# DINT-NSDI24/DINT

Hardware: AMD Instinct MI355X
Metric: Mtxn/s + p50/p99 batch latency, TATP (higher is better)
Workload: dtype u64

## Files before the change

### dint_amd/csrc/k_kv_dev.h

```cpp
#pragma once
#include <algorithm>
#include <cstddef>
#include <cstdlib>
#include <cstring>
#include <utility>
#include <vector>

#include "../../include/dint_abi.h"
#include "dint_kv.h"
#define KVB_SORT_INLINE
#include "dint_bins.h"
#include "log_ring.h"

template <int WL> struct Fmt;
template <> struct Fmt<DINT_WL_STORE> {
  static constexpr uint32_t MSG = 53, TYPE = 0, KEY = 1, VAL = 9, VER = 49, VS = 40;
  static constexpr bool HAS_TABLE = false;
  static constexpr uint32_t TABLE = 0;
};
template <> struct Fmt<DINT_WL_TATP> {
  static constexpr uint32_t MSG = 55, TYPE = 1, KEY = 3, VAL = 11, VER = 51, VS = 40;
  static constexpr bool HAS_TABLE = true;
  static constexpr uint32_t TABLE = 2;
};
// ... 2012 lines not shown
            uint32_t pos;
            if (fancy) {
              const int lw = top(mW & below), lwb = top((mW | mB) & below);
              const uint32_t w = wc + (uint32_t)__popcll(mW & below);
              const uint32_t jj = (lw < 0 ? jc : 0u) + (uint32_t)__popcll(mB & below & above(lw));
              const uint64_t mine = q == 0 ? mA[0] : q == 1 ? mA[1] : q == 2 ? mA[2] : mA[3];
              const bool follows = (mine & below & above(lwb)) != 0 || (lwb < 0 && ((af >> q) & 1u));
              pos = w * stride + (cl == 0 ? 0u : cl == 1 ? 3u * jj + (follows ? 1u : 0u) : cl == 2 ? 3u * jj + 2u : stride - 1u);
            } else {
              pos = 2u * (vc + (uint32_t)__popcll(mV & below)) + (cl ? 1u : 0u);
            }
            if (valid) Rpos[p] = (uint16_t)pos;
            const int tw = top(mW), twb = top(mW | mB);
            wc += (uint32_t)__popcll(mW);
            jc = (tw < 0 ? jc : 0u) + (uint32_t)__popcll(mB & above(tw));
            if (twb >= 0) af = 0;
#pragma unroll
            for (uint32_t i = 0; i < 4; i++) af |= (mA[i] & above(twb)) ? 1u << i : 0u;
            vc += (uint32_t)__popcll(mV);
          }
        }
      }
    }
    __syncthreads();
    for (uint32_t j = 0; j < ntile; j++) {
      const uint32_t p = j * KVB_T + t;
      const uint32_t pos = p < m ? Rpos[p] : 0xFFFFu;
      if (pos != 0xFFFFu) atomicOr(&Rbits[pos >> 5], 1u << (pos & 31));
    }
    {
      uint32_t mx = mylen;
      for (int d = 32; d > 0; d >>= 1) mx = max(mx, (uint32_t)__shfl_xor(mx, d, 64));
      if (lane == 0) Sred[wave] = mx;
      __syncthreads();
      tot = 0;
      for (uint32_t w = 0; w < KVB_W; w++) tot = max(tot, Sred[w]);
    }
    for (uint32_t rw = 0; rw * 32 < tot; rw++) {
      for (uint32_t bits = Rbits[rw]; bits; bits &= bits - 1) {
        const uint32_t r = rw * 32 + (uint32_t)__ffs((int)bits) - 1;
        nrounds++;
        for (uint32_t j = 0; j < ntile; j++) {
          const uint32_t p = j * KVB_T + t;
          if (p < m && Rpos[p] == r) {
            const uint64_t cur = Sk[p];
            const uint32_t gk = kv_cut_gk((uint32_t)(cur >> sh_g), bin, cut), table = kv_table_of(kv, gk);
            kv_do_request<WL>(rep + dint_view_off(V, k_idx(cur), F::MSG), k_type(cur), table, k_q(cur),
                              (uint64_t)(gk - kv->gk_base[table]), kv, stats);
          }
        }
        __builtin_amdgcn_fence(__ATOMIC_SEQ_CST, "workgroup");
        __syncthreads();
      }
    }
    }
    if (wtr && t == 0) { wtr[14] += nrounds; wtr[15] += 1; }
    KVB_STAMP(13);
    __builtin_amdgcn_fence(__ATOMIC_SEQ_CST, "workgroup");
    __syncthreads();
  }
#undef KVB_STAMP
}

#define KVR_LCAP 1024u
#define KVR_F 64u
#define KVR_NPMAX 64u
struct kvr_lds {
  uint4 rec[KVR_LCAP];
  uint32_t hist[KVR_F];
  uint32_t cur[KVR_F];
  uint32_t off[KVR_F + 1];
  uint32_t bigoff[KVR_F];
  uint2 chs[KVR_F];
  uint32_t nch;
  uint32_t cflag[KVR_F];
  uint64_t ckey[KVR_F], hrec[KVR_F];
};
__device__ static inline uint32_t kv_piece_of(uint32_t idx, uint32_t np, uint32_t inv_n) {
  const uint32_t p = (uint32_t)(((uint64_t)idx * np * inv_n) >> 32);
  return p < np ? p : np - 1;
}
#define KVQ_W 3u
enum : uint32_t { KVQ_SUB = 0, KVQ_PIECE = 1, KVQ_REM = 2, KVQ_SOLO = 3 };

__device__ static inline void kv_list_items(const kv_pass_args &A, uint32_t b, const kvr_lds &L, const uint2 *Sbig) {
  const uint32_t t = threadIdx.x & 63u;
  const uint2 bs = Sbig[t];
  uint32_t target = A.split_target;
  if (A.V.seg_cap) {
    uint32_t live = t < A.V.n_seg ? min(A.V.seg_cap, *(const uint32_t *)(A.V.cnt + (size_t)t * A.V.cnt_stride)) : 0u, tot;
    (void)wave_excl_scan_u32(live, &tot);
    if (tot < A.n) target = max(8u, (uint32_t)(((uint64_t)target * max(tot, 1u)) / A.n));
  }
  const uint32_t np0 = (bs.y + target - 1) / target;
  const bool hot = bs.y >= A.split_min && np0 <= A.np_max;
  const uint32_t np = hot ? np0 : 0u;
  const uint32_t nent = bs.y ? (np > 1 ? np + 1 : 1u) : 0u;
  uint32_t tot, at = wave_excl_scan_u32(nent, &tot);
  uint32_t base = 0;
  if (t == 0 && tot) base = atomicAdd(&A.big[3], tot);
  base = (uint32_t)__builtin_amdgcn_readfirstlane((int)base);
  at += base;
  const uint32_t bin = b + A.cut.P * t;
  if (nent && !hot) {
    kv_st_agent(A.bigq + KVQ_W * (size_t)at, make_uint4(bin, bs.x, bs.y, KVQ_SUB));
  } else if (nent) {
    uint64_t hk = L.ckey[t], hr = L.hrec[t];
    if (A.sb_pieces) {
      using F = Fmt<DINT_WL_SMALLBANK>;
      const uint32_t sh_g = 16 + A.cut.ibits;
      uint64_t smp[8];
#pragma unroll
      for (uint32_t j = 0; j < 8; j++) smp[j] = kv_ld_agent(&A.ovf[bs.x + (uint32_t)(((uint64_t)(2 * j + 1) * bs.y) >> 4)]);
      uint32_t best = 0, bj = 0;
#pragma unroll
      for (uint32_t j = 0; j < 8; j++) {
        uint32_t c = 0;
#pragma unroll
        for (uint32_t i = 0; i < 8; i++) c += (smp[i] >> sh_g) == (smp[j] >> sh_g) && pay_q(kv_rec_pay(smp[i])) == pay_q(kv_rec_pay(smp[j]));
        if (c > best) { best = c; bj = j; }
      }
      hr = smp[0];
#pragma unroll
      for (uint32_t j = 1; j < 8; j++) if (j == bj) hr = smp[j];
      const uint32_t hidx = (uint32_t)(hr >> 16) & (uint32_t)((1ull << A.cut.ibits) - 1ull);
      hk = ld_u64(A.rep + dint_view_off(A.V, hidx, F::MSG) + F::KEY);
    }
    for (uint32_t p = 0; p < nent; p++) {
      const uint32_t kind = np == 1 ? KVQ_SOLO : (p < np ? KVQ_PIECE : KVQ_REM);
      uint4 *q = A.bigq + KVQ_W * (size_t)(at + p);
      kv_st_agent(q, make_uint4(bin, bs.x, bs.y, kind | (p << 2) | (np << 10)));
      kv_st_agent(q + 1, make_uint4((uint32_t)hk, (uint32_t)(hk >> 32), at, 0u));
      kv_st_agent(q + 2, make_uint4((uint32_t)hr, (uint32_t)(hr >> 32), 0u, 0u));
    }
  }
  asm volatile("s_waitcnt vmcnt(0)" ::: "memory");
  for (uint32_t p = 0; p < nent; p++)
    if (at + p < DINT_KV_BIGQ_MAX) __hip_atomic_store(&A.bigrdy[at + p], A.seq, __ATOMIC_RELAXED, __HIP_MEMORY_SCOPE_AGENT);
  asm volatile("s_waitcnt vmcnt(0)" ::: "memory");
  if (t == 0) atomicAdd(&A.big[6], 1u);
}

template <int WL, uint32_t NT>
__device__ static inline void kv_coarse_bin(const kv_pass_args &A, const kv_dev *kv, uint32_t coarse, uint8_t *lds_raw,
                                            uint2 *Sbig ,
                                            uint32_t cnt, const uint4 &r0, const uint4 &r1, uint64_t *tr) {
  kvr_lds &L = *(kvr_lds *)lds_raw;
  const uint32_t t = threadIdx.x, lane = t & 63, wave = t >> 6;
  const kv_cut &cut = A.cut;
  const uint32_t C = cut.P, cap = A.cap, sh = 16 + cut.ibits;
  const uint32_t idx_mask = (uint32_t)((1ull << cut.ibits) - 1ull);
  const uint4 *__restrict__ recs = A.kbins + (size_t)coarse * cap;
  if (cnt == 0) {
    if (t == 0) atomicAdd(&A.big[6], 1u);
    return;
  }
  const uint32_t n_in = min(cnt, cap);
  const uint32_t novl = cnt > cap ? A.big[1] : 0u;
  if (t == 0) A.bin_cnt[coarse] = 0;
  auto for_each_record = [&](auto &&f) {
    if (t < n_in) f(r0);
    if (t + NT < n_in) f(r1);
    for (uint32_t k0 = 2 * NT; k0 < n_in; k0 += 8 * NT) {
      uint4 q4[8];
#pragma unroll
      for (uint32_t j = 0; j < 8; j++) {
// ... 100 lines not shown
    const uint4 r = has ? L.rec[ab.x + lane] : make_uint4(0, 0, 0, 0);
    const uint64_t key0 = u4_key(r), m = u4_meta(r);
    const uint32_t pay0 = kv_rec_pay(m);
    uint64_t w = ~0ull;
    if (has) w = ((m >> sh) << (15 + cut.ibits)) | ((uint64_t)pay_kh(pay0) << (6 + cut.ibits)) | ((uint64_t)((uint32_t)(m >> 16) & idx_mask) << 6) | lane;
    w = wave_sort_u64(w);
    uint64_t *ctr = (tr && ch == 0) ? tr + 2 : nullptr;
    if (ctr && lane == 0) tr[5] = __builtin_amdgcn_s_memrealtime();
    const bool valid = lane < c;
    const int src = (int)((uint32_t)w & 63u);
    const uint64_t key = shfl_u64(key0, src);
    const uint32_t pay = (uint32_t)__shfl((int)pay0, src, 64);
    const uint32_t gk = kv_cut_gk((uint32_t)(w >> (15 + cut.ibits)), coarse, cut), kh = (uint32_t)(w >> (6 + cut.ibits)) & 511u;
    const uint32_t idx = (uint32_t)(w >> 6) & idx_mask;
    kv_chunk<WL>(A.rep, valid, valid ? idx : 0, gk, kh, pay_type(pay), valid ? kv_table_of(kv, gk) : 0, pay_q(pay), key, kv, A.stats,
                 A.force_flags & 1, true, A.V, ctr);
  }
}

template <int WL>
__device__ __forceinline__ static void kv_resolve_role(const kv_pass_args &A, uint32_t b, kv_dev &Skv, uint8_t *Lraw, uint2 *Sbig) {
  constexpr uint32_t NT = KVB_T;
  const uint32_t t = threadIdx.x;
  uint64_t *tr = A.trace ? A.trace + 32 * (size_t)b : nullptr;
  if (tr && t == 0) tr[0] = __builtin_amdgcn_s_memrealtime();
  static_assert(sizeof(kv_dev) / 4 <= NT, "one word of the table descriptors per thread");
  const uint4 *__restrict__ recs = A.kbins + (size_t)b * A.cap;
  const uint4 r0 = t < A.cap ? recs[t] : make_uint4(0, 0, 0, 0);
  const uint4 r1 = t + NT < A.cap ? recs[t + NT] : make_uint4(0, 0, 0, 0);
  const uint32_t kvw = t < sizeof(kv_dev) / 4 ? kv_dev_word(A.kv, A.big, t) : 0u;
  const uint32_t cnt = A.bin_cnt[b];
  if (t < sizeof(kv_dev) / 4) ((uint32_t *)&Skv)[t] = kvw;
  if (t < KVR_F) {
    Sbig[t] = make_uint2(0u, 0u);
    kvr_lds &L = *(kvr_lds *)Lraw;
    L.hist[t] = 0; L.cur[t] = 0; L.cflag[t] = 0;
  }
  if (b == 0) {
    if (t < 16 || (t >= KV_CTL_INS && t < KV_CTL_END)) A.big_z[t] = 0;
    for (uint32_t k = t; k < 1024; k += NT) A.blk_pub_z[k] = 0;
  }
  __syncthreads();
  kv_dev_pend_set(Skv, A.pno);
  if (tr && t == 0) tr[1] = __builtin_amdgcn_s_memrealtime();
  kv_coarse_bin<WL, NT>(A, &Skv, b, Lraw, Sbig, cnt, r0, r1, tr);
  if (tr && t == 0) { tr[11] = tr[12] = __builtin_amdgcn_s_memrealtime(); tr[13] = b; }
}
template <int WL>
__global__ void __launch_bounds__(KVB_T, 4) k_kv_resolve(kv_multi_args M, uint32_t n_eng) {
  __shared__ kv_dev Skv;
  __shared__ __attribute__((aligned(16))) uint8_t Lraw[sizeof(kvr_lds)];
  __shared__ uint2 Sbig[KVR_F];
  uint32_t e = 0, b = blockIdx.x;
  while (e + 1 < n_eng && b >= M.e[e].cut.P) { b -= M.e[e].cut.P; e++; }
  kv_resolve_role<WL>(M.e[e], b, Skv, Lraw, Sbig);
}

__device__ static inline unsigned long long kvh_word(uint32_t seq, bool ok, uint32_t nwr, int lw_idx, int ll_acq) {
  return ((unsigned long long)(seq & 0x3FFFFFFFu) << 34) | ((unsigned long long)(ok ? 1u : 0u) << 33) | ((unsigned long long)nwr << 23) |
         (lw_idx >= 0 ? (1ull << 22) | ((unsigned long long)(uint32_t)lw_idx << 2) : 0ull) | (ll_acq >= 0 ? 2ull | (unsigned long long)(ll_acq & 1) : 0ull);
}
struct kvh_lds {
  uint32_t key[KVB_T];
  uint32_t idx[KVB_T];
  uint8_t typ[KVB_T];
  uint64_t rem[KVB_T];
  uint64_t all[KVB_T];
  uint16_t cs[KVB_T + 2];
  uint64_t Bw[KVB_W], Bl[KVB_W], Ba[KVB_W];
  unsigned long long pub[KVR_NPMAX + 1];
  uint32_t bad, timeout, nhot, nrem, nall, nsame, nbr, nch, too_big;
  uint32_t found, link, slot, ver0, la0, table;
  uint32_t rowv[10];
  uint32_t best;
  unsigned long long hkey;
  uint32_t ev_ver[KVB_T];
  int16_t ev_src[KVB_T];
  uint8_t ev_ex[KVB_T];
  uint32_t fin_ex, fin_ver, fin_multi, fin_miss, dupf;
  int fin_src;
  uint8_t qq[KVB_T];
  uint64_t Lq[4][KVB_W], Aq[4][KVB_W];
  uint32_t lockw, bestg, gbad;
};
template <int WL>
__device__ __forceinline__ static bool kv_rem_chunks(uint8_t *rep, const kv_cut cut2, const kv_dev *kv, uint32_t bin, uint64_t *R, uint32_t m,
                                                     kvh_lds &H, dint_dev_stats *__restrict__ stats, int force_rounds, const dint_view V,
                                                     bool sorted = false ) {
  using F = Fmt<WL>;
  const uint32_t t = threadIdx.x, lane = t & 63, wave = t >> 6;
  const uint32_t sh_g = 16 + cut2.ibits, sh_k = 7 + cut2.ibits, idx_mask = (uint32_t)((1ull << cut2.ibits) - 1ull);
  __syncthreads();
  if (!sorted) {
    const uint64_t mine = t < m ? kv_sort_key(R[t], cut2) : ~0ull;
    __syncthreads();
    R[t] = mine;
    __syncthreads();
    uint32_t N = 64;
    while (N < m) N <<= 1;
    kvb_sort_blocked<1>(R, N);
  }
  const uint64_t w = R[t];
  const bool head = t < m && (t == 0 || (R[t - 1] >> sh_g) != (w >> sh_g));
  const uint64_t hm = __ballot(head);
  if (lane == 0) H.Bw[wave] = hm;
  __syncthreads();
  if (t == 0) {
    uint32_t nch = 0, start = 0, prev = 0, big = 0;
    for (uint32_t wv = 0; wv < KVB_W; wv++)
      for (uint64_t mm = H.Bw[wv]; mm; mm &= mm - 1) {
        const uint32_t hp = wv * 64 + (uint32_t)__ffsll((unsigned long long)mm) - 1;
        if (hp == 0) continue;
        if (hp - start > 64) { H.cs[nch++] = (uint16_t)start; start = prev; big |= hp - start > 64; }
        prev = hp;
      }
    if (m - start > 64) { H.cs[nch++] = (uint16_t)start; start = prev; big |= m - start > 64; }
    H.cs[nch++] = (uint16_t)start;
    H.cs[nch] = (uint16_t)m;
    H.nch = nch; H.too_big = big;
  }
  __syncthreads();
  if (H.too_big) return false;
  const uint32_t nch = H.nch;
  for (uint32_t ch = wave; ch < nch; ch += KVB_W) {
    const uint32_t a = H.cs[ch], c = H.cs[ch + 1] - a;
    const bool valid = lane < c;
    const uint64_t wv = valid ? R[a + lane] : ~0ull;
    const uint32_t idx = valid ? (uint32_t)(wv >> 7) & idx_mask : 0, gk = kv_cut_gk((uint32_t)(wv >> sh_g), bin, cut2);
    const uint32_t pay = (uint32_t)wv & 0x7Fu;
    const uint64_t key = valid ? ld_u64(rep + dint_view_off(V, idx, F::MSG) + F::KEY) : 0;
    kv_chunk<WL>(rep, valid, idx, gk, (uint32_t)(wv >> sh_k) & 511u, pay_type(pay), valid ? kv_table_of(kv, gk) : 0, pay_q(pay), key, kv, stats,
                 force_rounds, ch + KVB_W >= nch, V);
  }
  __builtin_amdgcn_fence(__ATOMIC_SEQ_CST, "workgroup");
  __syncthreads();
  return true;
}
#define KVG_MAXW 24u
template <int WL>
__device__ __forceinline__ static bool kv_group_phases(uint8_t *rep, const kv_cut cut2, const kv_dev *kv, uint32_t bin, const uint64_t *R, uint32_t Gs,
                                                       uint32_t Ge, kvh_lds &H, dint_dev_stats *__restrict__ stats, const dint_view V) {
  using F = Fmt<WL>;
  const uint32_t t = threadIdx.x, lane = t & 63, wave = t >> 6, n = Ge - Gs;
  const uint32_t sh_g = 16 + cut2.ibits, idx_mask = (uint32_t)((1ull << cut2.ibits) - 1ull);
  auto is_set = [](uint32_t type) -> bool { return WL == DINT_WL_STORE ? type == 1 : (type == 12 || type == 13); };
  auto is_ins = [](uint32_t type) -> bool { return WL == DINT_WL_STORE ? type == 2 : (type == 18 || type == 19); };
  auto is_del = [](uint32_t type) -> bool { return WL == DINT_WL_TATP && (type == 22 || type == 23); };
  const uint32_t gk = kv_cut_gk((uint32_t)(R[Gs] >> sh_g), bin, cut2), table = kv_table_of(kv, gk);
  const kv_tab tb = kv->tab[table];
  const uint64_t bucket = (uint64_t)(gk - kv->gk_base[table]);
  uint8_t *ie = kv_entry_ptr(tb, bucket, KV_INLINE);
  __syncthreads();
  {
    const uint64_t w = t < n ? R[Gs + t] : 0;
    const uint32_t idx = (uint32_t)(w >> 7) & idx_mask, pay = (uint32_t)w & 0x7Fu;
    H.key[t] = t < n ? (idx << 9) | t : 0xFFFFFFFFu;
    H.typ[t] = (uint8_t)(pay_type(pay) & 0xFFu);
    H.qq[t] = (uint8_t)pay_q(pay);
    H.rem[t] = t < n ? ld_u64(rep + dint_view_off(V, idx, F::MSG) + F::KEY) : 0;
    if (t == 0) { H.gbad = 0; H.lockw = KV_LD(uint32_t, ie + KV_LOCKB_OFF); }
  }
  __syncthreads();
  kvb_sort_blocked_u32<1>(H.key, KVB_T);
  const uint32_t sk = H.key[t];
  const bool v = sk != 0xFFFFFFFFu;
  const uint32_t slot = sk & 511u, my_idx = sk >> 9, my_type = v ? H.typ[slot] : 0xFFu, my_q = v ? H.qq[slot] : 0u;
// ... 70 lines not shown
      }
    }
  }
  __builtin_amdgcn_fence(__ATOMIC_SEQ_CST, "workgroup");
  __syncthreads();
  return true;
}
template <int WL>
__device__ __forceinline__ static int kv_solo_item(uint8_t *rep, const kv_cut cut2, const kv_dev *kv, const uint4 d,
                                                   const uint64_t *__restrict__ ovf, uint64_t *__restrict__ ovf2,
                                                   dint_dev_stats *__restrict__ stats, int force_rounds, const dint_view V, uint8_t *lds_raw,
                                                   uint32_t *src, uint32_t *off, uint32_t *cnt, uint64_t *ttr,
                                                   bool preloaded = false ) {
  using F = Fmt<WL>;
  kvh_lds &H = *(kvh_lds *)lds_raw;
  const uint32_t t = threadIdx.x, lane = t & 63, wave = t >> 6;
  const uint32_t h = d.z;
  const uint32_t sh_g = 16 + cut2.ibits, sh_k = 7 + cut2.ibits, idx_mask = (uint32_t)((1ull << cut2.ibits) - 1ull);
  *src = 0; *off = d.y; *cnt = h;
  if (h > KVB_T) return 1;
  auto is_set = [](uint32_t type) -> bool { return WL == DINT_WL_STORE ? type == 1 : (type == 12 || type == 13); };
  auto is_ins = [](uint32_t type) -> bool { return WL == DINT_WL_STORE ? type == 2 : (type == 18 || type == 19); };
  auto is_del = [](uint32_t type) -> bool { return WL == DINT_WL_TATP && (type == 22 || type == 23); };
  __syncthreads();
  if (!preloaded) H.all[t] = t < h ? kv_sort_key(kv_ld_agent(&ovf[d.y + t]), cut2) : ~0ull;
  if (t == 0) { H.bad = 0; H.best = 0; H.bestg = 0; H.dupf = 0; }
  __syncthreads();
  {
    uint32_t N = 64;
    while (N < h) N <<= 1;
    kvb_sort_blocked<1>(H.all, N);
  }
  const uint64_t w = H.all[t];
  const bool valid = t < h;
  const uint64_t prevw = t ? H.all[t - 1] : 0;
  const bool head_k = valid && (t == 0 || (prevw >> sh_k) != (w >> sh_k));
  const bool head_g = valid && (t == 0 || (prevw >> sh_g) != (w >> sh_g));
  const uint64_t mk = __ballot(head_k), mg = __ballot(head_g);
  if (lane == 0) { H.Bw[wave] = mk; H.Bl[wave] = mg; }
  __syncthreads();
  auto next_head = [&](const uint64_t *M) -> uint32_t {
    uint32_t nxt = h;
    for (uint32_t wv = wave; wv < KVB_W && nxt == h; wv++) {
      uint64_t mm = M[wv];
      if (wv == wave) mm &= ~((2ull << lane) - 1ull);
      if (mm) nxt = wv * 64 + (uint32_t)__ffsll((unsigned long long)mm) - 1;
    }
    return nxt;
  };
  if (head_k) atomicMax(&H.best, ((next_head(H.Bw) - t) << 16) | t);
  if (head_g) atomicMax(&H.bestg, ((next_head(H.Bl) - t) << 16) | t);
  __syncthreads();
  const uint32_t L = H.best >> 16, P = H.best & 0xFFFFu;
  uint32_t Gs = H.bestg & 0xFFFFu, Ge = Gs + (H.bestg >> 16);
  if (L > 64) {
    Gs = 0;
    for (uint32_t wv = 0; wv < KVB_W; wv++) {
      uint64_t mm = H.Bl[wv];
      if (wv * 64 > P) break;
      if (wv == (P >> 6)) mm &= (2ull << (P & 63)) - 1ull;
      if (mm) Gs = wv * 64 + 63 - (uint32_t)__clzll((long long)mm);
    }
    Ge = h;
    for (uint32_t wv = P >> 6; wv < KVB_W && Ge == h; wv++) {
      uint64_t mm = H.Bl[wv];
      if (wv == (P >> 6)) mm &= ~((2ull << (P & 63)) - 1ull);
      if (mm) Ge = wv * 64 + (uint32_t)__ffsll((unsigned long long)mm) - 1;
    }
  }
  auto rest = [&](uint32_t lo, uint32_t len) -> int {
    const uint32_t c_rem = h - len;
    if (c_rem == 0) return 0;
    __syncthreads();
    if (valid && (t < lo || t >= lo + len)) H.rem[t < lo ? t : t - len] = w;
    if (t >= c_rem) H.rem[t] = ~0ull;
    __builtin_amdgcn_fence(__ATOMIC_SEQ_CST, "workgroup");
    if (kv_rem_chunks<WL>(rep, cut2, kv, d.x, H.rem, c_rem, H, stats, force_rounds, V, true)) return 0;
    if (ovf2 && t < c_rem) {
      const uint64_t sw = H.rem[t];
      ovf2[d.y + t] = ((sw >> sh_g) << sh_g) | ((uint64_t)((uint32_t)(sw >> 7) & idx_mask) << 16) | ((uint32_t)sw & 0x7Fu) | (((uint32_t)(sw >> sh_k) & 511u) << 7);
    }
    __builtin_amdgcn_fence(__ATOMIC_SEQ_CST, "workgroup");
    *src = 1; *off = d.y; *cnt = c_rem;
    return 1;
  };
  auto phases = [&]() -> int {
    if (!kv_group_phases<WL>(rep, cut2, kv, d.x, H.all, Gs, Ge, H, stats, V)) return 1;
    return rest(Gs, Ge - Gs);
  };
  if (L <= 64) {
    if (ttr && t == 0) ttr[30] = (uint64_t)(d.w & 0xFFFFu) | (1ull << 17) | ((uint64_t)L << 20) | ((uint64_t)h << 32);
    if (Ge - Gs <= 64) return kv_rem_chunks<WL>(rep, cut2, kv, d.x, H.all, h, H, stats, force_rounds, V, true) ? 0 : 1;
    return phases();
  }
  const uint64_t hw = H.all[P];
  const uint32_t hq = pay_q((uint32_t)hw & 0x7Fu);
  const bool v = valid && t >= P && t < P + L;
  const uint32_t my_idx = (uint32_t)(w >> 7) & idx_mask, my_type = valid ? pay_type((uint32_t)w & 0x7Fu) : 0xFFu;
  if (valid && !v && (w >> sh_g) == (hw >> sh_g) && (kv_struct_op<WL>(my_type) || (kv_lock_op<WL>(my_type) && pay_q((uint32_t)w & 0x7Fu) == hq))) atomicOr(&H.bad, kv_struct_op<WL>(my_type) ? 1u : 2u);
  const uint64_t my_key = v ? ld_u64(rep + dint_view_off(V, my_idx, F::MSG) + F::KEY) : 0;
  if (t == P) H.hkey = my_key;
  const bool setop = v && is_set(my_type), insop = v && is_ins(my_type), delop = v && is_del(my_type);
  const bool lk = v && kv_lock_op<WL>(my_type), aq = v && WL == DINT_WL_TATP && my_type == 1;
  if (v && !(kv_simple_op<WL>(my_type) || kv_struct_op<WL>(my_type))) atomicOr(&H.bad, 4u);
  const uint64_t bev = __ballot(setop || insop || delop), bl = __ballot(lk), ba = __ballot(aq), bst = __ballot(insop || delop);
  if (lane == 0) { H.Bw[wave] = bev; H.Bl[wave] = bl; H.Ba[wave] = ba; }
  if (bst && lane == 0) H.dupf = 1;
  H.idx[t] = my_idx;
  H.typ[t] = (uint8_t)(my_type & 0xFFu);
  __syncthreads();
  const uint64_t hkey = H.hkey;
  if (v && my_key != hkey) atomicOr(&H.bad, 8u);
  const bool structural = H.dupf != 0;
  __syncthreads();
  kv_hdr Hd;
  kv_tab tb;
  uint64_t bucket = 0;
  uint32_t table = 0;
  {
    const uint32_t gk = kv_cut_gk((uint32_t)(hw >> sh_g), d.x, cut2);
    table = kv_table_of(kv, gk);
    tb = kv->tab[table];
    bucket = (uint64_t)(gk - kv->gk_base[table]);
  }
  if (t == P) {
    kv_hdr_load(Hd, kv_entry_ptr(tb, bucket, KV_INLINE));
    const kv_where wh = kv_locate(tb, bucket, Hd, hkey);
    H.found = wh.found; H.link = wh.link; H.slot = wh.slot; H.ver0 = wh.ver;
    H.la0 = WL == DINT_WL_TATP ? (Hd.lockw >> (8 * hq)) & 0xFFu : 0u;
    if (wh.found) {
      const uint8_t *rv = kv_entry_ptr(tb, bucket, wh.link) + KV_VAL_OFF + wh.slot * F::VS;
#pragma unroll
      for (uint32_t k = 0; k < F::VS / 4; k++) H.rowv[k] = KV_LD(uint32_t, rv + 4 * k);
    }
    uint32_t ex = wh.found, ver = wh.ver, toggles = 0, miss = 0, e = 0;
    int sr = -1;
    const uint32_t plow = structural ? kv_pool_low(kv, table) : 0u;
    uint32_t bail = plow | ((structural && kv_has_dup(tb, bucket, Hd, hkey, wh)) ? 1u : 0u);
    for (uint32_t wv = 0; wv < KVB_W; wv++)
      for (uint64_t mm = H.Bw[wv]; mm; mm &= mm - 1) {
        const uint32_t p = wv * 64 + (uint32_t)__ffsll((unsigned long long)mm) - 1;
        const uint32_t ty = H.typ[p];
        if (!bail) {
          if (is_set(ty)) { if (ex) { ver++; sr = (int)p; } else if (WL != DINT_WL_STORE) miss++; }
          else if (is_ins(ty)) { if (ex) bail = 1; else { ex = 1; ver = 0; sr = (int)p; toggles++; } }
          else { if (ex) { ex = 0; toggles++; } else miss++; }
          H.ev_ex[e] = (uint8_t)ex; H.ev_ver[e] = ver; H.ev_src[e] = (int16_t)sr;
        }
        e++;
      }
    if (bail) atomicOr(&H.bad, 16u);
    H.fin_ex = ex; H.fin_ver = ver; H.fin_src = sr; H.fin_multi = toggles > 1; H.fin_miss = miss;
  }
  __syncthreads();
  if (ttr && t == 0) ttr[30] = (uint64_t)(d.w & 0xFFFFu) | ((uint64_t)(H.bad ? 0u : 1u) << 16) | ((uint64_t)(structural ? 1u : 0u) << 18) | ((uint64_t)(L & 0xFFFu) << 20) | ((uint64_t)(H.bad & 31u) << 56) | ((uint64_t)(h - L) << 32);
  if (H.bad) return phases();
  const uint32_t found = H.found, ver0 = H.ver0, la0 = H.la0;
  uint32_t ev_below = 0;
  int ll_below = -1, ll_tot = -1;
#pragma unroll
  for (uint32_t wv = 0; wv < KVB_W; wv++) {
    const uint64_t me = H.Bw[wv], ml = H.Bl[wv];
    const uint64_t meb = wv < wave ? me : (wv == wave ? me & lanemask_lt() : 0ull), mlb = wv < wave ? ml : (wv == wave ? ml & lanemask_lt() : 0ull);
    ev_below += (uint32_t)__popcll(meb);
    if (mlb) ll_below = (int)(wv * 64 + 63 - __clzll((long long)mlb));
    if (ml) ll_tot = (int)(wv * 64 + 63 - __clzll((long long)ml));
  }
// ... 201 lines not shown
    if (j != 0 || !do_piece) return 0;
    if (nbr || solo) { *src = 0; *off = d.y; *cnt = h; return 1; }
    const uint32_t nsame = H.nsame;
    __syncthreads();
    if (t == 0) H.nhot = 0;
    __syncthreads();
    for (uint32_t k0 = 0; k0 < h; k0 += KVB_T) {
      const uint32_t k = k0 + t;
      const uint64_t r = k < h ? kv_ld_agent(&ovf[d.y + k]) : 0;
      const bool same = k < h && (r >> sh_g) == (hrec >> sh_g) && pay_kh(kv_rec_pay(r)) == hkh;
      const uint64_t mm = __ballot(same);
      uint32_t at = 0;
      if (lane == 0 && mm) at = atomicAdd(&H.nhot, (uint32_t)__popcll(mm));
      at = (uint32_t)__builtin_amdgcn_readfirstlane((int)at) + (uint32_t)__popcll(mm & lanemask_lt());
      if (same) ovf2[d.y + (h - nsame) + at] = r;
    }
    __builtin_amdgcn_fence(__ATOMIC_SEQ_CST, "workgroup");
    *src = 1; *off = d.y + (h - nsame); *cnt = nsame;
    return 1;
  }
  if (c != 0) {
    uint32_t nw_before = 0, nw_all = 0;
    int lw_before = -1, la_before = -1, jw = -1, jl = -1, la_fin = -1;
    for (uint32_t k = 0; k < np; k++) {
      const unsigned long long w = H.pub[k];
      const uint32_t nwk = (uint32_t)(w >> 23) & 1023u;
      if (k < j) {
        nw_before += nwk;
        if ((w >> 22) & 1ull) lw_before = (int)((w >> 2) & 0xFFFFFu);
        if (w & 2ull) la_before = (int)(w & 1ull);
      }
      nw_all += nwk;
      if (nwk) jw = (int)k;
      if (w & 2ull) { jl = (int)k; la_fin = (int)(w & 1ull); }
    }
    const uint32_t found = H.found, ver0 = H.ver0, la0 = H.la0;
    const kv_tab tb = kv->tab[H.table];
    const uint32_t gk = kv_cut_gk((uint32_t)(hrec >> sh_g), d.x, cut2);
    const uint64_t bucket = (uint64_t)(gk - kv->gk_base[H.table]);
    uint8_t *row = kv_entry_ptr(tb, bucket, H.link) + KV_VAL_OFF + H.slot * F::VS;
    if (v) {
      uint8_t *msg = rep + dint_view_off(V, my_idx, F::MSG);
      uint32_t code;
      bool get = false;
      if (WL == DINT_WL_STORE) {
        code = my_type == 0 ? (found ? 3 : 7) : (found ? 5 : 7);
        get = my_type == 0 && found;
      } else {
        const int seen = ll_below >= 0 ? acq_at(ll_below) : (la_before >= 0 ? la_before : (int)la0);
        switch (my_type) {
          case 0: code = found ? 4 : 6; get = found != 0; break;
          case 1: code = seen ? 8 : 7; break;
          case 2: code = 9; break;
          case 12: code = 15; break;
          default: code = 16; break;
        }
      }
      if (get) {
        const int widx = lw_below >= 0 ? (int)H.idx[lw_below] : lw_before;
        if (widx >= 0) {
          kv_copy_words(msg + F::VAL, rep + dint_view_off(V, (uint32_t)widx, F::MSG) + F::VAL, F::VS);
        } else {
#pragma unroll
          for (uint32_t k = 0; k < F::VS / 4; k++) st_u32(msg + F::VAL + 4 * k, H.rowv[k]);
        }
        st_u32(msg + F::VER, ver0 + nw_before + wr_below);
      }
      msg[F::TYPE] = (uint8_t)code;
    }
    if (found && nw_all && (int)j == jw && (int)t == lw_tot) {
      kv_copy_words(row, rep + dint_view_off(V, my_idx, F::MSG) + F::VAL, F::VS);
      KV_ST(uint32_t, &kv_entry_hdr(tb, bucket, H.link)->ver[H.slot], ver0 + nw_all);
    }
    if (WL == DINT_WL_TATP && t == 0) {
      if ((int)j == jl && la_fin >= 0 && (uint32_t)la_fin != la0) KV_ST(uint8_t, kv_entry_ptr(tb, bucket, KV_INLINE) + KV_LOCKB_OFF + hq, (uint8_t)la_fin);
      if (!found && wr_tot) atomicAdd(&stats->missing_keys, (unsigned long long)wr_tot);
    }
  }
  if (c_rem == 0) return 0;
  __builtin_amdgcn_fence(__ATOMIC_SEQ_CST, "workgroup");
  if (c_rem <= KVB_T && kv_rem_chunks<WL>(rep, cut2, kv, d.x, H.rem, c_rem, H, stats, force_rounds, V)) return 0;
  __builtin_amdgcn_fence(__ATOMIC_SEQ_CST, "workgroup");
  *src = 1; *off = d.y; *cnt = c_rem;
  return 1;
}

template <int WL>
__device__ __forceinline__ static void kv_serial_group(uint8_t *rep, const kv_cut cut2, const kv_dev *kv, uint32_t bin, const uint64_t *R, uint32_t Gs,
                                                       uint32_t Ge, kvh_lds &H, dint_dev_stats *__restrict__ stats, const dint_view V) {
  using F = Fmt<WL>;
  const uint32_t t = threadIdx.x, n = Ge - Gs;
  const uint32_t sh_g = 16 + cut2.ibits, idx_mask = (uint32_t)((1ull << cut2.ibits) - 1ull);
  __syncthreads();
  {
    const uint64_t w = t < n ? R[Gs + t] : 0;
    const uint32_t idx = (uint32_t)(w >> 7) & idx_mask, pay = (uint32_t)w & 0x7Fu;
    H.key[t] = t < n ? (idx << 9) | t : 0xFFFFFFFFu;
    H.typ[t] = (uint8_t)(pay_type(pay) & 0xFFu);
    H.qq[t] = (uint8_t)pay_q(pay);
  }
  __syncthreads();
  kvb_sort_blocked_u32<1>(H.key, KVB_T);
  if (t == 0) {
    const uint32_t gk = kv_cut_gk((uint32_t)(R[Gs] >> sh_g), bin, cut2), table = kv_table_of(kv, gk);
    const uint64_t bucket = (uint64_t)(gk - kv->gk_base[table]);
    for (uint32_t p = 0; p < n; p++) {
      const uint32_t sk = H.key[p], slot = sk & 511u;
      kv_do_request<WL>(rep + dint_view_off(V, sk >> 9, F::MSG), H.typ[slot], table, H.qq[slot], bucket, kv, stats);
      __builtin_amdgcn_fence(__ATOMIC_SEQ_CST, "workgroup");
    }
  }
  __builtin_amdgcn_fence(__ATOMIC_SEQ_CST, "workgroup");
  __syncthreads();
}
template <int WL>
__device__ __forceinline__ static void kv_late_stretch(uint8_t *rep, const kv_cut cut2, const kv_dev *kv, uint32_t bin, uint32_t h, kvh_lds &H,
                                                       dint_dev_stats *__restrict__ stats, int force_rounds, const dint_view V) {
  const uint32_t t = threadIdx.x, lane = t & 63, wave = t >> 6;
  const uint32_t sh_g = 16 + cut2.ibits;
  for (;;) {
    uint32_t src = 0, off = 0, cnt = h;
    const int run = kv_solo_item<WL>(rep, cut2, kv, make_uint4(bin, 0u, h, KVQ_SOLO), nullptr, nullptr, stats, force_rounds, V, (uint8_t *)&H, &src, &off,
                                     &cnt, nullptr, true);
    if (!run) return;
    if (!(src == 1 && cnt < h)) break;
    __syncthreads();
    const uint64_t w = t < cnt ? H.rem[t] : ~0ull;
    __syncthreads();
    H.all[t] = w;
    h = cnt;
    __syncthreads();
  }
  uint32_t m = h;
  for (;;) {
    __syncthreads();
    const uint64_t w = H.all[t];
    const bool head_g = t < m && (t == 0 || (H.all[t - 1] >> sh_g) != (w >> sh_g));
    const uint64_t mg = __ballot(head_g);
    if (t == 0) H.bestg = 0;
    if (lane == 0) H.Bl[wave] = mg;
    __syncthreads();
    if (head_g) {
      uint32_t nxt = m;
      for (uint32_t wv = wave; wv < KVB_W && nxt == m; wv++) {
        uint64_t mm = H.Bl[wv];
        if (wv == wave) mm &= ~((2ull << lane) - 1ull);
        if (mm) nxt = wv * 64 + (uint32_t)__ffsll((unsigned long long)mm) - 1;
      }
      atomicMax(&H.bestg, ((nxt - t) << 16) | t);
    }
    __syncthreads();
    const uint32_t Gs = H.bestg & 0xFFFFu, len = H.bestg >> 16;
    if (len <= 64) {
      kv_rem_chunks<WL>(rep, cut2, kv, bin, H.all, m, H, stats, force_rounds, V, true);
      return;
    }
    if (force_rounds || !kv_group_phases<WL>(rep, cut2, kv, bin, H.all, Gs, Gs + len, H, stats, V))
      kv_serial_group<WL>(rep, cut2, kv, bin, H.all, Gs, Gs + len, H, stats, V);
    __syncthreads();
    const bool mv = t >= Gs + len && t < m;
    const uint64_t mw = mv ? H.all[t] : 0;
    __syncthreads();
    if (mv) H.all[t - len] = mw;
    if (t >= m - len && t < m) H.all[t] = ~0ull;
    m -= len;
    if (m == 0) return;
  }
// ... 289 lines not shown
      asm volatile("s_waitcnt vmcnt(0)" ::: "memory");
    }
    __syncthreads();
    if (t == 0) __hip_atomic_store(&pub[np], kvh_word(seq, all_ok, 0, -1, -1), __ATOMIC_RELAXED, __HIP_MEMORY_SCOPE_AGENT);
  }
  if (t == 0) H.pub[KSB_NPMAX] = spin_for(&pub[np]);
  __syncthreads();
  if (H.timeout) __builtin_trap();
  if (!((H.pub[KSB_NPMAX] >> 33) & 1ull)) {
    if (j != 0) return 0;
    if (t == 0) atomicAdd(&stats->late_requests, (unsigned long long)h);
    *src = 0; *off = d.y; *cnt = h;
    return 1;
  }
  const uint32_t solo_rem = solo ? H.nrem : 0u;
  auto done = [&]() -> int {
    if (!solo_rem) return 0;
    __builtin_amdgcn_fence(__ATOMIC_SEQ_CST, "workgroup");
    *src = 1; *off = d.y; *cnt = solo_rem;
    return 1;
  };
  if (t < KVB_W) H.G[t] = kv_ld_agent(&sbx[(size_t)(first + j) * KSB_WORDS + 4 * KVB_W + t]);
  if (t < np) H.pub[t] = __hip_atomic_load(&pub[t], __ATOMIC_RELAXED, __HIP_MEMORY_SCOPE_AGENT);
  __syncthreads();
  if (c == 0) return done();
  uint32_t nw_before = 0, nw_all = 0;
  int lw_before = -1, jw = -1;
  for (uint32_t k = 0; k < np; k++) {
    const unsigned long long w = H.pub[k];
    const uint32_t nwk = (uint32_t)(w >> 23) & 1023u;
    if (k < j) {
      nw_before += nwk;
      if ((w >> 22) & 1ull) lw_before = (int)((w >> 2) & 0xFFFFFu);
    }
    nw_all += nwk;
    if (nwk) jw = (int)k;
  }
  const uint32_t found = H.found, ver0 = H.ver0;
  uint32_t miss = 0;
  if (v && !foreign) {
    const bool granted = (H.G[wave] >> lane) & 1ull;
    uint32_t code;
    bool get = false;
    switch (my_type) {
      case 0: code = granted ? 7 : 8; get = granted; break;
      case 1: code = granted ? 9 : 10; get = granted; break;
      case 2: code = 11; break;
      case 3: code = 12; break;
      case 4: code = 13; miss = !found; break;
      case 5: code = 14; miss = !found; break;
      default: code = 18; get = true; break;
    }
    if (get && found) {
      const int widx = lw_below >= 0 ? (int)H.idx[lw_below] : lw_before;
      if (widx >= 0) {
        const uint8_t *fm = rep + dint_view_off(V, (uint32_t)widx, F::MSG) + F::VAL;
        const uint32_t a0 = ld_u32(fm), a1 = ld_u32(fm + 4);
        st_u32(msg + F::VAL, a0); st_u32(msg + F::VAL + 4, a1);
      } else {
        st_u32(msg + F::VAL, H.rowv[0]); st_u32(msg + F::VAL + 4, H.rowv[1]);
      }
      st_u32(msg + F::VER, ver0 + nw_before + wr_below);
    } else if (get && my_type != 17u) {
      miss = 1;
    }
    msg[F::TYPE] = (uint8_t)code;
  }
  {
    const uint64_t mm = __ballot(miss != 0);
    if (lane == 0 && mm) atomicAdd(&stats->missing_keys, (unsigned long long)__popcll(mm));
  }
  if (found && nw_all && (int)j == jw && (int)t == lw_tot) {
    uint8_t *row = kv_entry_ptr(tb, bucket, H.link) + KV_VAL_OFF + H.slot * F::VS;
    KV_ST(uint32_t, row, ld_u32(msg + F::VAL));
    KV_ST(uint32_t, row + 4, ld_u32(msg + F::VAL + 4));
    KV_ST(uint32_t, &kv_entry_hdr(tb, bucket, H.link)->ver[H.slot], ver0 + nw_all);
  }
  return done();
}

static_assert(sizeof(kvb_lds) + KVB_BM_BYTES + sizeof(kv_dev) <= 160 * 1024, "k_kv_big must fit the 160 KB of LDS of a gfx950 CU");
static_assert(sizeof(kvb_lds) + (KV_HOT_BM ? KV_HOT_BM_W * 10 : 16) + sizeof(kv_dev) <= 160 * 1024, "k_kv_big must fit the 160 KB of LDS of a gfx950 CU");
#define KVW_GRID 96u
template <int WL>
__device__ __forceinline__ static void kv_hot_role(const kv_pass_args &A, kv_dev &Skv, uint8_t *Lraw, uint32_t &Stk, uint32_t bx, uint32_t by) {
  const uint32_t t = threadIdx.x;
  if (t < sizeof(kv_dev) / 4) ((uint32_t *)&Skv)[t] = kv_dev_word(A.kv, A.big, t);
  __syncthreads();
  kv_dev_pend_set(Skv, A.pno);
  kv_cut cut2 = A.cut;
  cut2.P = A.cut.P * KVR_F;
  uint64_t *tr = A.trace ? A.trace + 2048 * 32 + 32 * (size_t)(by * KVB_GRID + bx) : nullptr;
  for (bool first = true;; first = false) {
    __syncthreads();
    if (t == 0) {
      const uint32_t i = atomicAdd(&A.big[4], 1u);
      uint32_t got = KV_NONE;
      for (uint32_t spins = 0; i < DINT_KV_BIGQ_MAX; spins++) {
        if (__hip_atomic_load(&A.bigrdy[i], __ATOMIC_RELAXED, __HIP_MEMORY_SCOPE_AGENT) == A.seq) { got = i; break; }
        if (__hip_atomic_load(&A.big[6], __ATOMIC_RELAXED, __HIP_MEMORY_SCOPE_AGENT) >= A.cut.P &&
            i >= __hip_atomic_load(&A.big[3], __ATOMIC_RELAXED, __HIP_MEMORY_SCOPE_AGENT)) break;
        if (spins > (1u << 22)) __builtin_trap();
        __builtin_amdgcn_s_sleep(4);
      }
      Stk = got;
    }
    __syncthreads();
    const uint32_t i = Stk;
    if (i == KV_NONE) break;
    const uint4 d = kv_ld_agent(A.bigq + KVQ_W * (size_t)i);
    uint32_t src = 0, off = d.y, cnt = d.z;
    uint64_t *ttr = first ? tr : nullptr;
    if (ttr && t == 0) { ttr[0] = __builtin_amdgcn_s_memrealtime(); ttr[2] = d.z; ttr[3] = d.x; ttr[30] = d.w; }
    int run = 1;
    if constexpr (WL == DINT_WL_SMALLBANK) {
      if ((d.w & 3u) != KVQ_SUB)
        run = kv_sb_item<WL>(A.rep, cut2, &Skv, d, kv_ld_agent(A.bigq + KVQ_W * (size_t)i + 1), kv_ld_agent(A.bigq + KVQ_W * (size_t)i + 2), A.ovf, A.ovf2,
                             A.hotpub, A.sbx, A.seq, A.inv_n, A.stats, A.V, Lraw, &src, &off, &cnt);
      if (run && src == 1 && cnt <= KVB_T) {
        kvh_lds &Hh = *(kvh_lds *)Lraw;
        __syncthreads();
        Hh.rem[t] = t < cnt ? A.ovf2[off + t] : 0ull;
        if (kv_rem_chunks<WL>(A.rep, cut2, &Skv, d.x, Hh.rem, cnt, Hh, A.stats, A.force_flags & 1, A.V)) run = 0;
      }
      if (run && t == 0) A.lateq[atomicAdd(&A.big[5], 1u)] = make_uint4(d.x, off, cnt, src);
    } else {
    if ((d.w & 3u) == KVQ_SOLO)
      run = kv_solo_item<WL>(A.rep, cut2, &Skv, d, A.ovf, A.ovf2, A.stats, A.force_flags & 1, A.V, Lraw, &src, &off, &cnt, ttr);
    else if ((d.w & 3u) != KVQ_SUB)
      run = kv_hot_item<WL>(A.rep, cut2, &Skv, d, kv_ld_agent(A.bigq + KVQ_W * (size_t)i + 1), kv_ld_agent(A.bigq + KVQ_W * (size_t)i + 2), A.ovf, A.ovf2,
                            A.hotpub, A.seq, A.inv_n, A.stats, A.force_flags & 1, A.V, Lraw, &src, &off, &cnt, ttr);
    if (run && t == 0) {
      A.lateq[atomicAdd(&A.big[5], 1u)] = make_uint4(d.x, off, cnt, src);
      atomicAdd(&A.stats->late_requests, (unsigned long long)cnt);
      atomicAdd(&A.stats->late_items[(d.w & 3u) == KVQ_SUB ? 0 : (d.w & 3u) == KVQ_SOLO ? 1 : 2], 1ULL);
    }
    }
    if (ttr && t == 0) ttr[1] = __builtin_amdgcn_s_memrealtime();
  }
}
template <int WL>
__global__ void __launch_bounds__(KVB_T, 4) k_kv_hot(kv_multi_args M) {
  __shared__ kv_dev Skv;
  __shared__ __attribute__((aligned(16))) uint8_t Lraw[sizeof(kvh_lds)];
  __shared__ uint32_t Stk;
  const kv_pass_args &A = M.e[blockIdx.y];
  if (blockIdx.x >= A.big[3]) return;
  kv_hot_role<WL>(A, Skv, Lraw, Stk, blockIdx.x, blockIdx.y);
}

template <int WL, int RPT>
__global__ void __launch_bounds__(KVB_T, 4) k_kv_hot_part(kv_pass_args H, kv_pass_args P) {
  constexpr size_t LB = sizeof(kvh_lds) > sizeof(kv_part_lds<RPT, KVB_T>) ? sizeof(kvh_lds) : sizeof(kv_part_lds<RPT, KVB_T>);
  __shared__ kv_dev Skv;
  __shared__ __attribute__((aligned(16))) uint8_t Lraw[LB];
  __shared__ uint32_t Stk;
  if (blockIdx.x < KVB_GRID) {
    if (blockIdx.x < H.big[3]) kv_hot_role<WL>(H, Skv, Lraw, Stk, blockIdx.x, 0);
    return;
  }
  const uint32_t b = blockIdx.x - KVB_GRID;
  if (b >= P.n_tiles) return;
  kv_part_body<WL, RPT, KVB_T>(P, *(kv_part_lds<RPT, KVB_T> *)Lraw, b == 0);
}

template <int WL, int RPT>
__global__ void __launch_bounds__(KVB_T, 4) k_kv_pass(kv_multi_args M, uint32_t n_eng, uint32_t sum_c, kv_multi_args PM ,
                                                       uint32_t max_tiles ,
                                                       uint32_t n_work ,
                                                       uint32_t part_first ) {
  constexpr size_t LW = sizeof(kvs_lds) > sizeof(kvh_lds) ? sizeof(kvs_lds) : sizeof(kvh_lds);
  constexpr size_t L1 = LW > sizeof(kvr_lds) ? LW : sizeof(kvr_lds);
  constexpr size_t LB = L1 > sizeof(kv_part_lds<RPT ? RPT : 1, KVB_T>) ? L1 : sizeof(kv_part_lds<RPT ? RPT : 1, KVB_T>);
  __shared__ kv_dev Skv;
  __shared__ __attribute__((aligned(16))) uint8_t Lraw[LB];
  __shared__ uint2 Sbig[KVR_F];
  __shared__ uint32_t Stk;
  uint32_t b = blockIdx.x;
  if (b < sum_c) {
    uint32_t e = 0;
    while (e + 1 < n_eng && b >= M.e[e].cut.P) { b -= M.e[e].cut.P; e++; }
    kv_resolve_role<WL>(M.e[e], b, Skv, Lraw, Sbig);
    return;
  }
  b -= sum_c;
  const uint32_t nw = n_work * n_eng, nt = RPT != 0 ? max_tiles * n_eng : 0u;
  const bool worker = part_first ? b >= nt : b < nw;
  if (worker) {
    if (part_first) b -= nt;
    if (b >= nw) return;
    const uint32_t e = b / n_work;
    kv_hot_role<WL>(M.e[e], Skv, Lraw, Stk, b - e * n_work, e);
    return;
  }
  if constexpr (RPT != 0) {
    if (!part_first) b -= nw;
    if (b >= nt) return;
    const uint32_t e = b / max_tiles, slot = b - e * max_tiles;
    const kv_pass_args &P = PM.e[e];
    if (slot >= P.n_tiles) return;
    kv_part_body<WL, RPT, KVB_T>(P, *(kv_part_lds<RPT, KVB_T> *)Lraw, slot == 0);
  }
}

template <int WL>
__global__ void __launch_bounds__(KVB_T, 1) k_kv_big(kv_multi_args M, uint32_t from_late) {
  static_assert(sizeof(kv_dev) + sizeof(kvb_lds) + (WL == DINT_WL_SMALLBANK ? KVB_BM_BYTES : 16) + 64 <= 160 * 1024, "k_kv_big's LDS must fit a gfx950 compute unit");
  __shared__ kv_dev Skv;
  __shared__ __attribute__((aligned(16))) uint8_t Lraw[sizeof(kvb_lds)];
  __shared__ __attribute__((aligned(16))) uint8_t Lbm[WL == DINT_WL_SMALLBANK ? KVB_BM_BYTES : KV_HOT_BM ? KV_HOT_BM_W * 10 : 16];
  __shared__ uint32_t Stk;
  const kv_pass_args &A = M.e[blockIdx.y];
  const uint32_t nq = from_late ? A.big[5] : A.big[3];
  if (blockIdx.x >= nq) return;
  const uint32_t t = threadIdx.x;
  if (t < sizeof(kv_dev) / 4) ((uint32_t *)&Skv)[t] = kv_dev_word(A.kv, A.big, t);
  __syncthreads();
  kv_dev_pend_set(Skv, A.pno);
  __syncthreads();
  kv_cut cut2 = A.cut;
  cut2.P = A.cut.P * KVR_F;
  if (from_late) {
    for (uint32_t i = blockIdx.x; i < nq; i += gridDim.x) {
      const uint4 d = A.lateq[i];
      const uint64_t *recs = (d.w ? (const uint64_t *)A.ovf2 : A.ovf) + d.y;
      kv_big_bin<WL>(A.rep, A.n, cut2, &Skv, d.x, recs, d.w || !A.ovf2 ? nullptr : A.ovf2 + d.y, d.z, A.stats, A.force_flags, A.V, Lraw, Lbm, nullptr);
    }
    return;
  }
  uint64_t *tr = A.trace ? A.trace + 2048 * 32 + 32 * (size_t)(blockIdx.y * KVB_GRID + blockIdx.x) : nullptr;
  for (bool first = true;; first = false) {
    __syncthreads();
    if (t == 0) Stk = atomicAdd(&A.big[4], 1u);
    __syncthreads();
    const uint32_t i = Stk;
    if (i >= nq) break;
    const uint4 d = A.bigq[KVQ_W * (size_t)i];
    uint32_t src = 0, off = d.y, cnt = d.z;
    uint64_t *ttr = first ? tr : nullptr;
    if (ttr && t == 0) { ttr[0] = __builtin_amdgcn_s_memrealtime(); ttr[2] = d.z; ttr[3] = d.x; ttr[30] = d.w; }
    const uint64_t t_in = tr ? __builtin_amdgcn_s_memrealtime() : 0ull;
// ... 99 lines not shown
```

Baseline: 3094.

## Rerun hot-item remainders in place as solo items instead of deferring them

When a hot or solo item leaves a small remainder, it now returns a distinct code. The block then rewrites its own queue slot as a SOLO item tagged RERUN and processes it again on its next iteration, instead of pushing the remainder to the late queue. A RERUN item reloads and re-sorts its keys from the overflow buffer before calling the solo path. The aim is to avoid the slower late pass for leftovers, at the cost of extra iterations, an agent-scope store plus release fence, and a new pending flag kept in shared scratch memory. The fused hot+part kernel opts out through a template flag.

```diff
diff --git a/dint_amd/csrc/k_kv_dev.h b/dint_amd/csrc/k_kv_dev.h
--- a/dint_amd/csrc/k_kv_dev.h
+++ b/dint_amd/csrc/k_kv_dev.h
@@ -2118,6 +2118,7 @@
 }
 #define KVQ_W 3u
 enum : uint32_t { KVQ_SUB = 0, KVQ_PIECE = 1, KVQ_REM = 2, KVQ_SOLO = 3 };
+#define KVQ_RERUN (1u << 24)
 
 __device__ static inline void kv_list_items(const kv_pass_args &A, uint32_t b, const kvr_lds &L, const uint2 *Sbig) {
   const uint32_t t = threadIdx.x & 63u;
@@ -2384,6 +2385,7 @@
   uint8_t qq[KVB_T];
   uint64_t Lq[4][KVB_W], Aq[4][KVB_W];
   uint32_t lockw, bestg, gbad;
+  uint32_t pend;
 };
 template <int WL>
 __device__ __forceinline__ static bool kv_rem_chunks(uint8_t *rep, const kv_cut cut2, const kv_dev *kv, uint32_t bin, uint64_t *R, uint32_t m,
@@ -2620,7 +2622,7 @@
     }
     __builtin_amdgcn_fence(__ATOMIC_SEQ_CST, "workgroup");
     *src = 1; *off = d.y; *cnt = c_rem;
-    return 1;
+    return 2;
   };
   auto phases = [&]() -> int {
     if (!kv_group_phases<WL>(rep, cut2, kv, d.x, H.all, Gs, Ge, H, stats, V)) return 1;
@@ -2988,7 +2990,7 @@
   if (c_rem <= KVB_T && kv_rem_chunks<WL>(rep, cut2, kv, d.x, H.rem, c_rem, H, stats, force_rounds, V)) return 0;
   __builtin_amdgcn_fence(__ATOMIC_SEQ_CST, "workgroup");
   *src = 1; *off = d.y; *cnt = c_rem;
-  return 1;
+  return 2;
 }
 
 template <int WL>
@@ -3444,7 +3446,7 @@
 static_assert(sizeof(kvb_lds) + KVB_BM_BYTES + sizeof(kv_dev) <= 160 * 1024, "k_kv_big must fit the 160 KB of LDS of a gfx950 CU");
 static_assert(sizeof(kvb_lds) + (KV_HOT_BM ? KV_HOT_BM_W * 10 : 16) + sizeof(kv_dev) <= 160 * 1024, "k_kv_big must fit the 160 KB of LDS of a gfx950 CU");
 #define KVW_GRID 96u
-template <int WL>
+template <int WL, bool RERUN = true >
 __device__ __forceinline__ static void kv_hot_role(const kv_pass_args &A, kv_dev &Skv, uint8_t *Lraw, uint32_t &Stk, uint32_t bx, uint32_t by) {
   const uint32_t t = threadIdx.x;
   if (t < sizeof(kv_dev) / 4) ((uint32_t *)&Skv)[t] = kv_dev_word(A.kv, A.big, t);
@@ -3453,9 +3455,13 @@
   kv_cut cut2 = A.cut;
   cut2.P = A.cut.P * KVR_F;
   uint64_t *tr = A.trace ? A.trace + 2048 * 32 + 32 * (size_t)(by * KVB_GRID + bx) : nullptr;
+  kvh_lds &Hp = *(kvh_lds *)Lraw;
+  if (RERUN && WL != DINT_WL_SMALLBANK && t == 0) Hp.pend = 0;
   for (bool first = true;; first = false) {
     __syncthreads();
-    if (t == 0) {
+    bool draw = t == 0;
+    if (RERUN && WL != DINT_WL_SMALLBANK && t == 0) { draw = Hp.pend == 0; Hp.pend = 0; }
+    if (draw) {
       const uint32_t i = atomicAdd(&A.big[4], 1u);
       uint32_t got = KV_NONE;
       for (uint32_t spins = 0; i < DINT_KV_BIGQ_MAX; spins++) {
@@ -3487,15 +3493,28 @@
       }
       if (run && t == 0) A.lateq[atomicAdd(&A.big[5], 1u)] = make_uint4(d.x, off, cnt, src);
     } else {
-    if ((d.w & 3u) == KVQ_SOLO)
-      run = kv_solo_item<WL>(A.rep, cut2, &Skv, d, A.ovf, A.ovf2, A.stats, A.force_flags & 1, A.V, Lraw, &src, &off, &cnt, ttr);
+    if ((d.w & 3u) == KVQ_SOLO) {
+      const bool rr = RERUN && (d.w & KVQ_RERUN) != 0;
+      if (rr) Hp.all[t] = t < d.z ? kv_sort_key(kv_ld_agent(&A.ovf2[d.y + t]), cut2) : ~0ull;
+      run = kv_solo_item<WL>(A.rep, cut2, &Skv, d, A.ovf, A.ovf2, A.stats, A.force_flags & 1, A.V, Lraw, &src, &off, &cnt, ttr, rr);
+    }
     else if ((d.w & 3u) != KVQ_SUB)
       run = kv_hot_item<WL>(A.rep, cut2, &Skv, d, kv_ld_agent(A.bigq + KVQ_W * (size_t)i + 1), kv_ld_agent(A.bigq + KVQ_W * (size_t)i + 2), A.ovf, A.ovf2,
                             A.hotpub, A.seq, A.inv_n, A.stats, A.force_flags & 1, A.V, Lraw, &src, &off, &cnt, ttr);
     if (run && t == 0) {
-      A.lateq[atomicAdd(&A.big[5], 1u)] = make_uint4(d.x, off, cnt, src);
-      atomicAdd(&A.stats->late_requests, (unsigned long long)cnt);
-      atomicAdd(&A.stats->late_items[(d.w & 3u) == KVQ_SUB ? 0 : (d.w & 3u) == KVQ_SOLO ? 1 : 2], 1ULL);
+      uint4 *q = A.bigq + KVQ_W * (size_t)i;
+      const uint4 &d0 = d;
+      const bool rerun = RERUN && (d0.w & KVQ_RERUN) != 0;
+      const uint32_t kind = rerun ? (d0.w >> 20) & 3u : d0.w & 3u;
+      if (RERUN && run == 2 && cnt <= KVB_T && cnt < d0.z) {
+        kv_st_agent(q, make_uint4(d0.x, off, cnt, KVQ_SOLO | KVQ_RERUN | (kind << 20)));
+        __builtin_amdgcn_fence(__ATOMIC_RELEASE, "agent");
+        Hp.pend = 1;
+      } else {
+        A.lateq[atomicAdd(&A.big[5], 1u)] = make_uint4(d0.x, off, cnt, rerun ? 1u : src);
+        atomicAdd(&A.stats->late_requests, (unsigned long long)cnt);
+        atomicAdd(&A.stats->late_items[kind == KVQ_SUB ? 0 : kind == KVQ_SOLO ? 1 : 2], 1ULL);
+      }
     }
     }
     if (ttr && t == 0) ttr[1] = __builtin_amdgcn_s_memrealtime();
@@ -3518,7 +3537,7 @@
   __shared__ __attribute__((aligned(16))) uint8_t Lraw[LB];
   __shared__ uint32_t Stk;
   if (blockIdx.x < KVB_GRID) {
-    if (blockIdx.x < H.big[3]) kv_hot_role<WL>(H, Skv, Lraw, Stk, blockIdx.x, 0);
+    if (blockIdx.x < H.big[3]) kv_hot_role<WL, false>(H, Skv, Lraw, Stk, blockIdx.x, 0);
     return;
   }
   const uint32_t b = blockIdx.x - KVB_GRID;
```

Result: no change. 3089 (-0.2%).
